# geopolars/geopolars

Hardware: AMD Instinct MI355X
Metric: predicate evals/sec (10M pts x 1k polys point-in-polygon) (higher is better)
Workload: dtype f64

## Files before the change

geopolars_amd/csrc/gpk_pipflow.hip:

```cpp
#include "gpk_pipshared.h"

namespace gpk {

constexpr int FLOW_P_MAX = 8;
constexpr int FLOW_BLOCK = 1024, FLOW_W = FLOW_BLOCK / 64;
constexpr int FLOW_ITEMS = 128;
constexpr int FLOW_PASS_AT = 40;
constexpr int FLOW_MAX_TILES = 1536;
constexpr int FLOW_ID_BITS = 22;
constexpr uint32_t FLOW_DEAD = 0xFFFFFFFFu;
constexpr uint32_t FLOW_MULTI = 0x80000000u;
constexpr uint32_t FLOW_PEND = FLOW_MULTI;
static_assert(64 * FLOW_P_MAX == 512, "an entry keeps the row within its tile in 9 bits");
static_assert(FLOW_MAX_TILES <= (1 << 14), "FlowItem::loc keeps the tile in 14 bits");

struct FlowItem {
    double px, py;
    uint32_t aux;
    uint32_t loc;
};
static_assert(sizeof(FlowItem) == 24, "list slot");

#ifdef GPK_TILE_TRACE
#define FLOW_STAMP(i)                                                                                                    \
    do {                                                                                                                 \
        if (h.stats && lane == 0 && wave % 5 == 0 && blockIdx.x < 900u) h.stats[8 + (blockIdx.x * 4 + wave / 5) * 16 + (i)] = wall_clock64(); \
    } while (0)
#if GPK_TILE_TRACE == 2
#define FLOW_PHASE(i)                                        \
    do {                                                     \
        asm volatile("s_waitcnt vmcnt(0) lgkmcnt(0)" ::: "memory"); \
        const unsigned long long _n = wall_clock64();        \
        g_phase[i] += _n - g_last;                           \
        g_last = _n;                                         \
    } while (0)
#define FLOW_PHASE_ARGS , unsigned long long (&g_phase)[6], unsigned long long& g_last
#define FLOW_PHASE_PASS , g_phase, g_last
#else
#define FLOW_PHASE(i) do {} while (0)
#define FLOW_PHASE_ARGS
#define FLOW_PHASE_PASS
#endif
#else
#define FLOW_STAMP(i) do {} while (0)
#define FLOW_PHASE(i) do {} while (0)
#define FLOW_PHASE_ARGS
#define FLOW_PHASE_PASS
#endif

#define H_COLD(field) (kernel_arg_at<decltype(ChainHot::field)>((uint32_t)offsetof(ChainHot, field)))
#define T_COLD(field) (kernel_arg_at<decltype(FusedTail::field)>((uint32_t)(sizeof(ChainHot) + offsetof(FusedTail, field))))
static_assert(sizeof(ChainHot) % 8 == 0, "FusedTail follows ChainHot in the argument segment");

__device__ __forceinline__ uint32_t cvt_u32_sat(double v) {
    uint32_t r;
    asm("v_cvt_u32_f64 %0, %1" : "=v"(r) : "v"(v));
    return r;
}
__device__ __forceinline__ void wave_lds_fence() {
    __builtin_amdgcn_fence(__ATOMIC_RELEASE, "wavefront");
    __builtin_amdgcn_wave_barrier();
    __builtin_amdgcn_fence(__ATOMIC_ACQUIRE, "wavefront");
}

__device__ __forceinline__ void ring_edge_flat(double sx, double sy, double ex, double ey, double cx, double cy, int& wn, bool& on, bool& unsure) {
    const bool up = sy <= cy && ey >= cy, down = sy > cy && ey <= cy;
    const bool left = cx < fmin(sx, ex), within = !left && cx <= fmax(sx, ex);
    const double detleft = (sx - cx) * (ey - cy), detright = (sy - cy) * (ex - cx);
    const double det = detleft - detright;
    const double errbound = 3.3306690738754716e-16 * (fabs(detleft) + fabs(detright));
    const bool opposite = (detleft > 0.0 && detright <= 0.0) || (detleft < 0.0 && detright >= 0.0) || detleft == 0.0;
    const bool certain = opposite || fabs(det) >= errbound;
    const bool eval = (up || down) && within;
    unsure |= eval && !certain;
    on |= eval && certain && det == 0.0;
    wn += (up && ey != cy && (left || (within && det > 0.0))) ? 1 : 0;
    wn -= (down && (left || (within && det < 0.0))) ? 1 : 0;
}

__device__ __forceinline__ void flow_settle(const ChainHot& h, uint32_t* s_ttot, uint32_t t, uint32_t slot, uint32_t row, uint32_t li, uint32_t cnt,
                                            uint32_t first) {
    if (cnt == 0u) {
        h.pool[slot] = FLOW_DEAD;
        if (h.counts) h.counts[row] = 0u;
        atomicSub(&s_ttot[t], 1u);
    } else if (cnt == 1u) {
        h.pool[slot] = (first << 9) | li;
    } else {
        h.pool[slot] = FLOW_MULTI | (cnt << 9) | li;
        if (h.counts) h.counts[row] = cnt;
        atomicAdd(&s_ttot[t], cnt - 1u);
    }
}

template <int TS>
__device__ __forceinline__ void flow_exact_pass(const ChainHot& h, FlowItem* items, uint32_t& n_list, int lane, uint32_t* s_ttot, uint32_t tile0) {
    const uint32_t n = n_list < 64u ? n_list : 64u;
    wave_lds_fence();
    const bool act = (uint32_t)lane < n;
    double qx = 0.0, qy = 0.0;
    uint32_t hd = 0u, loc = 0u;
    if (act) {
        const FlowItem* it = items + lane;
        qx = it->px;
        qy = it->py;
        hd = it->aux;
        loc = it->loc;
    }
    const int count = (int)(hd & HCHAIN_COUNT_MASK);
    const double2* __restrict__ v = H_COLD(chain_xy) + (hd >> HCHAIN_START_SHIFT);
    const int i1 = count < 1 ? count : 1, i2 = count < 2 ? count : 2, i3 = count < 3 ? count : 3, i4 = count < 4 ? count : 4;
    double2 a0 = v[0], a1 = v[i1], a2 = v[i2], a3 = v[i3], a4 = v[i4];
    asm volatile("" : "+v"(a0.x), "+v"(a0.y), "+v"(a1.x), "+v"(a1.y), "+v"(a2.x), "+v"(a2.y), "+v"(a3.x), "+v"(a3.y), "+v"(a4.x), "+v"(a4.y));
    int wn = ((int)(hd << (28 - HCHAIN_BASE_SHIFT))) >> 28;
    bool unsure = false, on = false;
    ring_edge_flat(a0.x, a0.y, a1.x, a1.y, qx, qy, wn, on, unsure);
    ring_edge_flat(a1.x, a1.y, a2.x, a2.y, qx, qy, wn, on, unsure);
    ring_edge_flat(a2.x, a2.y, a3.x, a3.y, qx, qy, wn, on, unsure);
    ring_edge_flat(a3.x, a3.y, a4.x, a4.y, qx, qy, wn, on, unsure);
    if (count > 4) {
        double ax = a4.x, ay = a4.y;
        for (int j = 4; j < count; ++j) {
            const double2 b = v[j + 1];
            on |= dev::ring_edge_filtered(ax, ay, b.x, b.y, qx, qy, wn, unsure);
            ax = b.x;
            ay = b.y;
        }
    }
    const bool walk = act && (count == 0 || unsure);
    const bool inside = !on && wn != 0;
    const uint32_t t = loc >> 18, li = loc & 511u;
    const uint32_t slot = ((tile0 + t) << TS) + ((loc >> 9) & 511u), row = ((tile0 + t) << TS) + li;
    if (act && !walk && !inside) flow_settle(h, s_ttot, t, slot, row, li, 0u, 0u);
    unsigned long long wm = __ballot(walk);
#ifdef GPK_TILE_TRACE
    unsigned long long* const stats = nullptr;
#else
    unsigned long long* const stats = H_COLD(stats);
#endif
    if (stats) {
        const unsigned long long edges = wave_sum_u64((unsigned long long)(act ? count : 0));
        if (lane == 0) {
            atomicAdd(&stats[0], (unsigned long long)n);
            atomicAdd(&stats[1], edges);
            if (wm) atomicAdd(&stats[2], (unsigned long long)__popcll(wm));
        }
    }
    while (wm) {
        const int j = __builtin_ctzll(wm);
        wm &= wm - 1ull;
        const double x = __shfl(qx, j, 64), y = __shfl(qy, j, 64);
        const unsigned long long cf = chain_generic_row_first_call(H_COLD(cold), x, y, lane);
        if (lane == j) flow_settle(h, s_ttot, t, slot, row, li, (uint32_t)cf, (uint32_t)(cf >> 32));
    }
    n_list -= n;
    if (n_list) {
        FlowItem keep{};
        if ((uint32_t)lane < n_list) keep = items[64 + lane];
        wave_lds_fence();
        if ((uint32_t)lane < n_list) items[lane] = keep;
    }
    wave_lds_fence();
}

typedef uint32_t u32x4 __attribute__((ext_vector_type(4)));

static __device__ __noinline__ void flow_settle_pending(const double2* pts_xy, const ChainCold* cold, uint32_t* pool, uint32_t* counts, unsigned long long* stats,
                                                        uint32_t* s_ttot, uint32_t t, uint32_t tile, uint32_t n_ent, int lane, int ts) {
    asm volatile("s_waitcnt vmcnt(0)" ::: "memory");
    uint32_t* seg = pool + ((size_t)tile << ts);
    for (uint32_t i = 0; i < n_ent; i += 64u) {
        const uint32_t e = i + (uint32_t)lane < n_ent ? __hip_atomic_load(seg + i + lane, __ATOMIC_RELAXED, __HIP_MEMORY_SCOPE_AGENT) : 0u;
        unsigned long long pm = __ballot((e & ~511u) == FLOW_PEND);
        while (pm) {
            const int j = __builtin_ctzll(pm);
            pm &= pm - 1ull;
            const uint32_t li = (uint32_t)__shfl((int)e, j, 64) & 511u, row = (tile << ts) + li, slot = i + (uint32_t)j;
            const double2 q = pts_xy[row];
            const unsigned long long cf = chain_generic_row_first_call(cold, q.x, q.y, lane);
            const uint32_t cnt = (uint32_t)cf, first = (uint32_t)(cf >> 32);
            if (lane == 0) {
                if (stats) atomicAdd(&stats[2], 1ull);
                if (cnt == 0u) {
                    seg[slot] = FLOW_DEAD;
                    if (counts) counts[row] = 0u;
                    atomicSub(&s_ttot[t], 1u);
                } else if (cnt == 1u) {
                    seg[slot] = (first << 9) | li;
                } else {
                    seg[slot] = FLOW_MULTI | (cnt << 9) | li;
                    if (counts) counts[row] = cnt;
                    atomicAdd(&s_ttot[t], cnt - 1u);
                }
            }
        }
    }
}

template <bool SIMPLE, bool FULL, int P>
__device__ __forceinline__ void flow_tile(const ChainHot& h, const uint2* s_mask, const uint32_t* s_rec0, FlowItem* items, uint32_t& n_list, uint32_t t,
                                          uint32_t tile0, int lane, uint32_t* s_tcand, uint32_t* s_ttot FLOW_PHASE_ARGS) {
    constexpr int S = PIP_SUB, FLOW_TILE = 64 * P, TS = P == 8 ? 9 : (P == 4 ? 8 : (P == 2 ? 7 : 6));
    static_assert(P == 1 || P == 2 || P == 4 || P == 8, "tile sizes");
    static_assert(S == 8, "the sub-cell arithmetic below is written for 8 x 8 sub-cells");
    asm volatile("" : "+v"(lane));
    const uint32_t tile = tile0 + t;
    const int64_t base = (int64_t)tile * FLOW_TILE;
    const int64_t n_points = FULL ? 0 : H_COLD(n_points);
    const uint32_t rem = FULL ? (uint32_t)FLOW_TILE : (uint32_t)(n_points - base < (int64_t)FLOW_TILE ? n_points - base : (int64_t)FLOW_TILE);
    double px[P], py[P];
    {
        const double2* __restrict__ tile_xy = h.pts_xy + base;
        static_for<P>([&](auto K) {
            constexpr int k = decltype(K)::value;
            double2 v = make_double2(NAN, NAN);
            if (FULL || ((uint32_t)(k * 64 + lane) < rem && dev::valid_row(H_COLD(pts_validity), base + k * 64 + lane))) v = dev::load_stream(tile_xy + (k * 64 + lane));
            px[k] = v.x;
            py[k] = v.y;
        });
    }
    GPK_SCHED_FENCE();
    FLOW_PHASE(1);
    const int logR = h.logR;
    const uint32_t sub_max = ((uint32_t)S << logR) - 1u;
    uint32_t sidx4[(P + 3) / 4], gw[P];
    u32x4 rec[P];
    static_for<(P + 3) / 4>([&](auto J) { sidx4[decltype(J)::value] = 0u; });
    uint32_t sxs[P], sys_[P], r0s[P];
    uint2 ms[P];
    static_for<P>([&](auto K) {
        constexpr int k = decltype(K)::value;
        uint32_t sx = cvt_u32_sat((px[k] - h.rx0) * h.inv_fw_s), sy = cvt_u32_sat((py[k] - h.ry0) * h.inv_fh_s);
        sx = sx < sub_max ? sx : sub_max;
        sy = sy < sub_max ? sy : sub_max;
        const uint32_t at = ((sy >> 3) << (logR - 5)) + (sx >> 8);
        ms[k] = s_mask[at];
        r0s[k] = s_rec0[at];
        sxs[k] = sx;
        sys_[k] = sy;
    });
    GPK_SCHED_FENCE();
    static_for<P>([&](auto K) {
        constexpr int k = decltype(K)::value;
        const uint32_t sx = sxs[k], sy = sys_[k], bit = (sx >> 3) & 31u;
        const bool real = !__builtin_isunordered(px[k], py[k]);
        const bool has = real && ((ms[k].x >> bit) & 1u) != 0u;
        const bool want = real && !has && ((ms[k].y >> bit) & 1u) != 0u;
        sidx4[k / 4] |= (((sy & 3u) << 3) | (sx & 7u)) << (8 * (k % 4));
        rec[k] = u32x4{0u, 0u, 0u, 0u};
        gw[k] = 0u;
        if (has) {
            const uint32_t w = r0s[k] + (uint32_t)__popc(__builtin_amdgcn_ubfe(ms[k].x, 0u, bit));
            rec[k] = *reinterpret_cast<const u32x4*>(h.half + (2u * w + ((sy >> 2) & 1u)));
        }
        if (want) gw[k] = h.cell[((sy >> 3) << logR) + (sx >> 3)];
    });
    GPK_SCHED_FENCE();
    FLOW_PHASE(2);
    uint32_t run = 0u, n_new = 0u;
    bool pend = false;
    uint32_t* const tile_counts = h.counts ? h.counts + base : nullptr;
    uint32_t* const tile_pool = h.pool + ((size_t)tile << TS);
    static_for<P>([&](auto K) {
        constexpr int k = decltype(K)::value;
        const uint32_t li = (uint32_t)(k * 64 + lane);
        const uint32_t s5 = (sidx4[k / 4] >> (8 * (k % 4))) & 31u;
        const uint32_t lw = (s5 & 16u) ? rec[k].y : rec[k].x;
        const uint32_t lab = (lw >> (2u * (s5 & 15u))) & 3u;
        uint32_t r = lab ? (rec[k].z & 0x3FFFFFFFu) : CODE_NONE;
        const uint32_t g = gw[k];
        const bool single = (g & 0xC0000001u) == 0x40000000u;
        if (single) r = (g >> 1) & 0x1FFFFFFFu;
        const bool walk = g != 0u && !single;
        if (!SIMPLE) {
            if (r != CODE_NONE) {
                const uint32_t geom = h.part_geom ? h.part_geom[r] : r;
                r = dev::valid_row(h.polys_validity, geom) ? geom : CODE_NONE;
            }
        }
        if (walk) r = 0u;
        const bool mine = FULL || li < rem;
        const bool cand = mine && r != CODE_NONE;
        bool listed = cand && (lab >= 2u || walk);
        const unsigned long long mcand = __ballot(cand);
        const uint32_t rank = run + lanes_below(mcand);
        uint32_t e = (r << 9) | li;
        unsigned long long ml = __ballot(listed);
        if (ml) {
            if (__builtin_expect(n_list + n_new + (uint32_t)__popcll(ml) > (uint32_t)FLOW_ITEMS, 0)) {
                if (listed && n_list + n_new + lanes_below(ml) >= (uint32_t)FLOW_ITEMS) {
                    listed = false;
                    e = FLOW_PEND | li;
                }
                ml = __ballot(listed);
                pend = true;
            }
            if (listed) {
                FlowItem* it = items + (n_list + n_new + lanes_below(ml));
                it->px = px[k];
                it->py = py[k];
                it->aux = walk ? 0u : rec[k].w;
                it->loc = (t << 18) | (rank << 9) | li;
            }
            n_new += (uint32_t)__popcll(ml);
        }
        if (tile_counts && mine) dev::store_stream(tile_counts + li, cand ? 1u : 0u);
        if (cand) tile_pool[rank] = e;
        run += (uint32_t)__popcll(mcand);
        GPK_SCHED_FENCE();
    });
    if (lane == 0) {
        s_tcand[t] = run;
        s_ttot[t] = run;
    }
    n_list += n_new;
    FLOW_PHASE(3);
    if (__builtin_expect(pend, 0)) flow_settle_pending(h.pts_xy, H_COLD(cold), h.pool, h.counts, H_COLD(stats), s_ttot, t, tile, run, lane, TS);
}

__device__ __forceinline__ void flow_emit_chunk(const ChainHot& h, uint32_t e, uint32_t row0, uint32_t pt0, unsigned long long* out64, uint32_t room, uint32_t& done,
                                                int lane) {
    const bool live = e != FLOW_DEAD;
    const bool multi = live && (e & FLOW_MULTI) != 0u;
    const unsigned long long mm = __ballot(multi);
    if (__builtin_expect(mm == 0ull, 1)) {
        const unsigned long long m = __ballot(live);
        const uint32_t at = done + lanes_below(m);
        if (live && at < room) __builtin_nontemporal_store(((unsigned long long)(e >> 9) << 32) | (unsigned long long)(row0 + (e & 511u)), out64 + at);
        done += (uint32_t)__popcll(m);
        return;
    }
    const uint32_t n_out = !live ? 0u : (multi ? (e >> 9) & ((1u << FLOW_ID_BITS) - 1u) : 1u);
    uint32_t incl = n_out;
#pragma unroll
    for (int o = 1; o < 64; o <<= 1) {
        const uint32_t v = __shfl_up(incl, o, 64);
        if (lane >= o) incl += v;
    }
    const uint32_t at = done + incl - n_out;
    if (live && !multi && at < room) __builtin_nontemporal_store(((unsigned long long)(e >> 9) << 32) | (unsigned long long)(row0 + (e & 511u)), out64 + at);
    unsigned long long wm = mm;
    while (wm) {
        const int j = __builtin_ctzll(wm);
        wm &= wm - 1ull;
        const uint32_t lj = (uint32_t)__shfl((int)e, j, 64) & 511u, aj = (uint32_t)__shfl((int)at, j, 64);
        const double2 q = h.pts_xy[pt0 + lj];
        chain_generic_row_call(H_COLD(cold), q.x, q.y, lane, reinterpret_cast<uint2*>(out64 + aj), aj < room ? room - aj : 0u, row0 + lj);
    }
    done += (uint32_t)__shfl((int)incl, 63, 64);
}

template <bool SIMPLE, int P>
__global__ __launch_bounds__(FLOW_BLOCK) void pip_tile_flow_kernel(ChainHot h, FusedTail tail) {
    constexpr int WORDS = PIP_ROUTE_RMAX * PIP_ROUTE_RMAX / 32, W = FLOW_W, TS = P == 8 ? 9 : (P == 4 ? 8 : (P == 2 ? 7 : 6));
    __shared__ uint2 s_mask[WORDS];
    __shared__ uint32_t s_rec0[WORDS];
    __shared__ FlowItem s_items[W][FLOW_ITEMS];
    __shared__ uint32_t s_tcand[FLOW_MAX_TILES], s_ttot[FLOW_MAX_TILES];
    __shared__ uint32_t s_next, s_next2, s_wg, s_wgtot, s_gave_up;
    __shared__ unsigned long long s_part[W];
    const int lane = threadIdx.x & 63, wave = __builtin_amdgcn_readfirstlane(threadIdx.x >> 6);
    FLOW_STAMP(0);
    unsigned long long my_ticket = 0ull;
    if (threadIdx.x == 0) my_ticket = __hip_atomic_fetch_add(T_COLD(ticket), 1ull, __ATOMIC_RELAXED, __HIP_MEMORY_SCOPE_AGENT);
    {
        const int R = H_COLD(R), words = R * R / 32;
        const uint4* __restrict__ src = reinterpret_cast<const uint4*>(H_COLD(route));
        for (int i = threadIdx.x; i < words; i += FLOW_BLOCK) {
            const uint4 rw = src[i];
            s_mask[i] = make_uint2(rw.x, rw.y);
            s_rec0[i] = rw.z;
        }
    }
    FLOW_STAMP(1);
    if (threadIdx.x == 0) {
        s_wg = (uint32_t)(my_ticket - T_COLD(ticket_base));
        s_next = 0u;
        s_next2 = 0u;
        s_gave_up = 0u;
    }
    __syncthreads();
    const uint32_t wg = __builtin_amdgcn_readfirstlane(s_wg);
    const uint32_t T0 = (uint32_t)((int64_t)wg * H_COLD(n_tiles) / (int64_t)gridDim.x), T1 = (uint32_t)((int64_t)(wg + 1u) * H_COLD(n_tiles) / (int64_t)gridDim.x);
    const uint32_t nt = T1 - T0;
    const bool want_pairs = T_COLD(pairs) != nullptr;
    FLOW_STAMP(2);
    const uint32_t nf = (int64_t)T1 <= (int64_t)H_COLD(n_full_tiles) ? nt : ((int64_t)T0 >= (int64_t)H_COLD(n_full_tiles) ? 0u : (uint32_t)(H_COLD(n_full_tiles) - (int32_t)T0));
    uint32_t n_list = 0u;
#ifdef GPK_TILE_TRACE
    int n_mine = 0;
#if GPK_TILE_TRACE == 2
    unsigned long long g_phase[6] = {0ull, 0ull, 0ull, 0ull, 0ull, 0ull}, g_last = wall_clock64();
#endif
#endif
    auto draw = [&](uint32_t* counter) -> uint32_t {
        __builtin_amdgcn_wave_barrier();
        const uint32_t d = __hip_atomic_fetch_add(counter, 1u, __ATOMIC_RELAXED, __HIP_MEMORY_SCOPE_WORKGROUP);
        return __builtin_amdgcn_readfirstlane(d) >> 6;
    };
    {
        uint32_t t = draw(&s_next);
        while (t < nf) {
            const uint32_t tn = draw(&s_next);
            FLOW_PHASE(4);
            if (n_list >= (uint32_t)FLOW_PASS_AT) flow_exact_pass<TS>(h, s_items[wave], n_list, lane, s_ttot, T0);
            FLOW_PHASE(0);
            flow_tile<SIMPLE, true, P>(h, s_mask, s_rec0, s_items[wave], n_list, t, T0, lane, s_tcand, s_ttot FLOW_PHASE_PASS);
            t = tn;
#if defined(GPK_TILE_TRACE) && GPK_TILE_TRACE != 2
            if (n_mine < 6) FLOW_STAMP(3 + n_mine);
            ++n_mine;
#endif
        }
    }
    for (;;) {
        const uint32_t t = draw(&s_next2) + nf;
        if (t >= nt) break;
        if (n_list >= (uint32_t)FLOW_PASS_AT) flow_exact_pass<TS>(h, s_items[wave], n_list, lane, s_ttot, T0);
        flow_tile<SIMPLE, false, P>(h, s_mask, s_rec0, s_items[wave], n_list, t, T0, lane, s_tcand, s_ttot FLOW_PHASE_PASS);
    }
    while (n_list) flow_exact_pass<TS>(h, s_items[wave], n_list, lane, s_ttot, T0);
#if defined(GPK_TILE_TRACE) && GPK_TILE_TRACE == 2
    FLOW_PHASE(5);
    if (h.stats && lane == 0 && wave % 5 == 0 && blockIdx.x < 900u)
        for (int i = 0; i < 6; ++i) h.stats[8 + (blockIdx.x * 4 + wave / 5) * 16 + 3 + i] = g_phase[i];
#endif
    FLOW_STAMP(9);
    __syncthreads();
    FLOW_STAMP(10);
    constexpr int EM_C = P < 4 ? P : 4, EM_T = 24 / EM_C;
    uint32_t ent[EM_T][EM_C], cand[EM_T];
    auto em_request = [&](uint32_t first) {
        static_for<EM_T>([&](auto Rr) {
            constexpr int r = decltype(Rr)::value;
            const uint32_t et = first + (uint32_t)(r * W);
            cand[r] = et < nt && want_pairs ? s_tcand[et] : 0u;
            cand[r] = __builtin_amdgcn_readfirstlane(cand[r]);
            const uint32_t* seg = h.pool + ((size_t)(T0 + et) << TS);
            static_for<EM_C>([&](auto Cc) {
                constexpr int c = decltype(Cc)::value;
                ent[r][c] = FLOW_DEAD;
                if ((uint32_t)(c * 64 + lane) < cand[r]) ent[r][c] = seg[c * 64 + lane];
            });
        });
    };
    em_request((uint32_t)wave);
    if (wave == 0) {
        uint32_t carry = 0u;
        for (uint32_t c0 = 0; c0 < nt; c0 += 64u) {
            const uint32_t v = c0 + (uint32_t)lane < nt ? s_ttot[c0 + lane] : 0u;
            uint32_t incl = v;
#pragma unroll
            for (int o = 1; o < 64; o <<= 1) {
                const uint32_t a = __shfl_up(incl, o, 64);
                if (lane >= o) incl += a;
            }
            if (c0 + (uint32_t)lane < nt) s_ttot[c0 + lane] = carry + incl - v;
            carry += (uint32_t)__shfl((int)incl, 63, 64);
        }
        if (lane == 0) s_wgtot = carry;
    }
    __syncthreads();
    const unsigned long long wg_tot = (unsigned long long)s_wgtot;
    const unsigned long long epoch = T_COLD(epoch);
    unsigned long long* const slots = T_COLD(slots);
    if (threadIdx.x == 0) __hip_atomic_store(&slots[wg], (epoch << FUSED_TOTAL_BITS) | wg_tot, __ATOMIC_RELAXED, __HIP_MEMORY_SCOPE_AGENT);
    unsigned long long acc = 0;
    bool gave_up = false;
    for (unsigned b = threadIdx.x; b < wg; b += FLOW_BLOCK) {
        unsigned long long v;
        uint32_t spins = 0;
        while (((v = __hip_atomic_load(&slots[b], __ATOMIC_RELAXED, __HIP_MEMORY_SCOPE_AGENT)) >> FUSED_TOTAL_BITS) != epoch) {
            __builtin_amdgcn_s_sleep(8);
            if (++spins > FUSED_SPIN_LIMIT) {
                gave_up = true;
                break;
            }
        }
        acc += v & ((1ull << FUSED_TOTAL_BITS) - 1ull);
    }
    if (gave_up) __hip_atomic_store(&s_gave_up, 1u, __ATOMIC_RELAXED, __HIP_MEMORY_SCOPE_WORKGROUP);
    acc = wave_sum_u64(acc);
    if (lane == 0) s_part[wave] = acc;
    __syncthreads();
    const bool lost = s_gave_up != 0u;
    unsigned long long base_off = 0;
#pragma unroll
    for (int w = 0; w < W; ++w) base_off += s_part[w];
    if ((wg == gridDim.x - 1 || lost) && threadIdx.x == 0) {
        unsigned long long* const lostp = T_COLD(lost);
        if (lost) __hip_atomic_store(lostp, epoch, __ATOMIC_RELAXED, __HIP_MEMORY_SCOPE_AGENT);
        const bool any_lost = lost || __hip_atomic_load(lostp, __ATOMIC_RELAXED, __HIP_MEMORY_SCOPE_AGENT) == epoch;
        unsigned long long* const grand = T_COLD(grand);
        unsigned long long* const grand_host = T_COLD(grand_host);
        *grand = any_lost ? FUSED_LOST : base_off + wg_tot;
        if (grand_host) *grand_host = any_lost ? FUSED_LOST : base_off + wg_tot;
    }
    FLOW_STAMP(11);
    if (!want_pairs || lost) return;
    unsigned long long* const pairs64 = reinterpret_cast<unsigned long long*>(T_COLD(pairs));
    const int64_t capacity = T_COLD(capacity);
    const uint32_t left_base = T_COLD(left_base);
    for (uint32_t first = (uint32_t)wave; first < nt; first += (uint32_t)(EM_T * W)) {
        if (first != (uint32_t)wave) em_request(first);
        static_for<EM_T>([&](auto Rr) {
            constexpr int r = decltype(Rr)::value;
            const uint32_t et = first + (uint32_t)(r * W);
            if (cand[r]) {
                const unsigned long long off = base_off + (unsigned long long)s_ttot[et];
                unsigned long long* const out64 = pairs64 + off;
                const int64_t left = capacity - (int64_t)off;
                const uint32_t room = left <= 0 ? 0u : (left > (int64_t)0xFFFFFFFFll ? 0xFFFFFFFFu : (uint32_t)left);
                const uint32_t pt0 = (T0 + et) << TS, row0 = pt0 + left_base;
                uint32_t done = 0u;
                static_for<EM_C>([&](auto Cc) {
                    constexpr int c = decltype(Cc)::value;
                    if ((uint32_t)(c * 64) < cand[r]) flow_emit_chunk(h, ent[r][c], row0, pt0, out64, room, done, lane);
                });
                if (EM_C * 64 < 64 * P) {
                    const uint32_t* seg = h.pool + ((size_t)(T0 + et) << TS);
                    for (uint32_t i = (uint32_t)(EM_C * 64); i < cand[r]; i += 64u) {
                        const uint32_t e = i + (uint32_t)lane < cand[r] ? seg[i + lane] : FLOW_DEAD;
                        flow_emit_chunk(h, e, row0, pt0, out64, room, done, lane);
                    }
                }
            }
        });
    }
    FLOW_STAMP(12);
}

int pip_flow_points_per_lane(int64_t n_left_rows, int64_t n_right_geoms, int32_t R, int wgs) {
    if (R < 32 || R > PIP_ROUTE_RMAX || wgs < 1) return 0;
    if (n_right_geoms >= (int64_t)((1u << FLOW_ID_BITS) - 1u)) return 0;
    if (n_left_rows >= (int64_t)0xFFFFFE00ll) return 0;
    static const int forced = [] {
        const char* e = getenv("GPK_FLOW_P");
        return e ? atoi(e) : 0;
    }();
    const int64_t waves = (int64_t)wgs * FLOW_W;
    for (int p = FLOW_P_MAX; p >= 1; p >>= 1) {
        const int64_t n_tiles = (n_left_rows + 64 * p - 1) / (64 * p);
        if ((n_tiles + wgs - 1) / wgs > (int64_t)FLOW_MAX_TILES) return p == FLOW_P_MAX ? 0 : 2 * p;
        if (forced ? p == forced : (n_tiles >= waves || p == 1)) return p;
    }
    return 1;
}
size_t pip_flow_pool_bytes(int64_t n_left_rows) { return sizeof(uint32_t) * (size_t)((n_left_rows + 511) / 512) * 512u; }

template <int P>
static int32_t launch_pip_flow_p(const ChainHot& hot, const FusedTail& tail, int wgs, hipStream_t s) {
    if (hot.part_geom == nullptr && hot.polys_validity == nullptr)
        GPK_LAUNCH("gpk_pip_tile", (pip_tile_flow_kernel<true, P>), dim3((unsigned)wgs), dim3(FLOW_BLOCK), 0, s, hot, tail);
    else
        GPK_LAUNCH("gpk_pip_tile", (pip_tile_flow_kernel<false, P>), dim3((unsigned)wgs), dim3(FLOW_BLOCK), 0, s, hot, tail);
    return GPK_OK;
}
int32_t launch_pip_flow(const ChainHot& hot, const FusedTail& tail, int wgs, int points_per_lane, hipStream_t s) {
    switch (points_per_lane) {
        case 8: return launch_pip_flow_p<8>(hot, tail, wgs, s);
        case 4: return launch_pip_flow_p<4>(hot, tail, wgs, s);
        case 2: return launch_pip_flow_p<2>(hot, tail, wgs, s);
        case 1: return launch_pip_flow_p<1>(hot, tail, wgs, s);
    }
    return fail(GPK_ERR_INVALID_ARGUMENT, "spatial_join: %d points per lane", points_per_lane);
}

}
```

Before: 115100 billion.

## Split exact pass into issue/finish to overlap edge loads with tile point loads

Splits the per-tile flow into a point-load request and a decide step. The deferred exact pass is split into an issue phase and a finish phase: the issue phase compacts the list and issues loads of up to four chain edges for short-chain items, then the next tile's point loads are issued, and the finish phase evaluates those edges. Items whose chains are longer, and results that are unsure, are pushed back onto the list for the full exact pass. This is meant to hide global-memory latency of the edge fetches behind the streaming point loads, at the cost of extra register pressure and added list-compaction work.

```diff
diff --git a/geopolars_amd/csrc/gpk_pipflow.hip b/geopolars_amd/csrc/gpk_pipflow.hip
--- a/geopolars_amd/csrc/gpk_pipflow.hip
+++ b/geopolars_amd/csrc/gpk_pipflow.hip
@@ -155,12 +155,139 @@
     }
     n_list -= n;
     if (n_list) {
-        FlowItem keep{};
-        if ((uint32_t)lane < n_list) keep = items[64 + lane];
+        const bool more = (uint32_t)lane < n_list;
+        double kx = 0.0, ky = 0.0;
+        uint32_t kaux = 0u, kloc = 0u;
+        if (more) {
+            const FlowItem* it = items + 64 + lane;
+            kx = it->px;
+            ky = it->py;
+            kaux = it->aux;
+            kloc = it->loc;
+        }
         wave_lds_fence();
-        if ((uint32_t)lane < n_list) items[lane] = keep;
+        if (more) {
+            FlowItem* it = items + lane;
+            it->px = kx;
+            it->py = ky;
+            it->aux = kaux;
+            it->loc = kloc;
+        }
     }
     wave_lds_fence();
+}
+
+struct FlowPass {
+    double2 a0, a1, a2, a3, a4;
+    double qx, qy;
+    uint32_t hd, loc;
+};
+constexpr uint32_t FLOW_SLOW_AT = 16;
+
+template <int TS>
+__device__ __forceinline__ void flow_pass_issue(const ChainHot& h, FlowItem* items, uint32_t& n_list, int lane, uint32_t* s_ttot, uint32_t tile0, FlowPass& ps) {
+    const uint32_t n = n_list < 64u ? n_list : 64u;
+    wave_lds_fence();
+    const bool act = (uint32_t)lane < n;
+    double qx = 0.0, qy = 0.0;
+    uint32_t aux = 0u, loc = 0u;
+    if (act) {
+        const FlowItem* it = items + lane;
+        qx = it->px;
+        qy = it->py;
+        aux = it->aux;
+        loc = it->loc;
+    }
+    const bool fast = act && (aux & HCHAIN_COUNT_MASK) - 1u < 4u;
+    const bool slow = act && !fast;
+    const unsigned long long ms = __ballot(slow);
+    const uint32_t rest = n_list - n, ns = (uint32_t)__popcll(ms);
+    if (rest | ns) {
+        const bool more = (uint32_t)lane < rest;
+        double kx = 0.0, ky = 0.0;
+        uint32_t kaux = 0u, kloc = 0u;
+        if (more) {
+            const FlowItem* it = items + 64 + lane;
+            kx = it->px;
+            ky = it->py;
+            kaux = it->aux;
+            kloc = it->loc;
+        }
+        wave_lds_fence();
+        if (slow) {
+            FlowItem* it = items + lanes_below(ms);
+            it->px = qx;
+            it->py = qy;
+            it->aux = aux;
+            it->loc = loc;
+        }
+        if (more) {
+            FlowItem* it = items + ns + lane;
+            it->px = kx;
+            it->py = ky;
+            it->aux = kaux;
+            it->loc = kloc;
+        }
+        wave_lds_fence();
+    }
+    n_list = ns + rest;
+    ps.qx = qx;
+    ps.qy = qy;
+    ps.hd = fast ? aux : 0u;
+    ps.loc = loc;
+    if (__builtin_expect(ns >= FLOW_SLOW_AT, 0)) flow_exact_pass<TS>(h, items, n_list, lane, s_ttot, tile0);
+    const int count = (int)(ps.hd & HCHAIN_COUNT_MASK);
+    const double2* __restrict__ v = H_COLD(chain_xy) + (ps.hd >> HCHAIN_START_SHIFT);
+    const int i1 = count < 1 ? count : 1, i2 = count < 2 ? count : 2, i3 = count < 3 ? count : 3;
+    ps.a0 = v[0];
+    ps.a1 = v[i1];
+    ps.a2 = v[i2];
+    ps.a3 = v[i3];
+    ps.a4 = v[count];
+}
+
+template <int TS>
+__device__ __forceinline__ void flow_pass_finish(const ChainHot& h, FlowItem* items, uint32_t& n_list, int lane, uint32_t* s_ttot, uint32_t tile0, FlowPass& ps) {
+    double2 a0 = ps.a0, a1 = ps.a1, a2 = ps.a2, a3 = ps.a3, a4 = ps.a4;
+    asm volatile("" : "+v"(a0.x), "+v"(a0.y), "+v"(a1.x), "+v"(a1.y), "+v"(a2.x), "+v"(a2.y), "+v"(a3.x), "+v"(a3.y), "+v"(a4.x), "+v"(a4.y));
+    const uint32_t hd = ps.hd, loc = ps.loc;
+    const double qx = ps.qx, qy = ps.qy;
+    const bool act = hd != 0u;
+    int wn = ((int)(hd << (28 - HCHAIN_BASE_SHIFT))) >> 28;
+    bool unsure = false, on = false;
+    ring_edge_flat(a0.x, a0.y, a1.x, a1.y, qx, qy, wn, on, unsure);
+    ring_edge_flat(a1.x, a1.y, a2.x, a2.y, qx, qy, wn, on, unsure);
+    ring_edge_flat(a2.x, a2.y, a3.x, a3.y, qx, qy, wn, on, unsure);
+    ring_edge_flat(a3.x, a3.y, a4.x, a4.y, qx, qy, wn, on, unsure);
+    const bool redo = act && unsure;
+    const bool inside = !on && wn != 0;
+    const uint32_t t = loc >> 18, li = loc & 511u;
+    const uint32_t slot = ((tile0 + t) << TS) + ((loc >> 9) & 511u), row = ((tile0 + t) << TS) + li;
+    if (act && !redo && !inside) flow_settle(h, s_ttot, t, slot, row, li, 0u, 0u);
+#ifdef GPK_TILE_TRACE
+    unsigned long long* const stats = nullptr;
+#else
+    unsigned long long* const stats = H_COLD(stats);
+#endif
+    if (stats) {
+        const unsigned long long settled = __ballot(act && !redo);
+        const unsigned long long edges = wave_sum_u64((unsigned long long)(hd & HCHAIN_COUNT_MASK));
+        if (lane == 0) {
+            atomicAdd(&stats[0], (unsigned long long)__popcll(settled));
+            atomicAdd(&stats[1], edges);
+        }
+    }
+    const unsigned long long mr = __ballot(redo);
+    if (__builtin_expect(mr != 0ull, 0)) {
+        if (redo) {
+            FlowItem* it = items + (n_list + lanes_below(mr));
+            it->px = qx;
+            it->py = qy;
+            it->aux = 0u;
+            it->loc = loc;
+        }
+        n_list += (uint32_t)__popcll(mr);
+    }
 }
 
 typedef uint32_t u32x4 __attribute__((ext_vector_type(4)));
@@ -197,28 +324,35 @@
     }
 }
 
+template <bool FULL, int P>
+__device__ __forceinline__ void flow_tile_request(const ChainHot& h, uint32_t t, uint32_t tile0, int lane, double (&px)[P], double (&py)[P]) {
+    constexpr int FLOW_TILE = 64 * P;
+    static_assert(P == 1 || P == 2 || P == 4 || P == 8, "tile sizes");
+    asm volatile("" : "+v"(lane));
+    const int64_t base = (int64_t)(tile0 + t) * FLOW_TILE;
+    const int64_t n_points = FULL ? 0 : H_COLD(n_points);
+    const uint32_t rem = FULL ? (uint32_t)FLOW_TILE : (uint32_t)(n_points - base < (int64_t)FLOW_TILE ? n_points - base : (int64_t)FLOW_TILE);
+    const double2* __restrict__ tile_xy = h.pts_xy + base;
+    static_for<P>([&](auto K) {
+        constexpr int k = decltype(K)::value;
+        double2 v = make_double2(NAN, NAN);
+        if (FULL || ((uint32_t)(k * 64 + lane) < rem && dev::valid_row(H_COLD(pts_validity), base + k * 64 + lane))) v = dev::load_stream(tile_xy + (k * 64 + lane));
+        px[k] = v.x;
+        py[k] = v.y;
+    });
+    GPK_SCHED_FENCE();
+}
+
 template <bool SIMPLE, bool FULL, int P>
-__device__ __forceinline__ void flow_tile(const ChainHot& h, const uint2* s_mask, const uint32_t* s_rec0, FlowItem* items, uint32_t& n_list, uint32_t t,
-                                          uint32_t tile0, int lane, uint32_t* s_tcand, uint32_t* s_ttot FLOW_PHASE_ARGS) {
+__device__ __forceinline__ void flow_tile_decide(const ChainHot& h, const uint2* s_mask, const uint32_t* s_rec0, FlowItem* items, uint32_t& n_list, uint32_t t,
+                                                 uint32_t tile0, int lane, uint32_t* s_tcand, uint32_t* s_ttot, double (&px)[P], double (&py)[P] FLOW_PHASE_ARGS) {
     constexpr int S = PIP_SUB, FLOW_TILE = 64 * P, TS = P == 8 ? 9 : (P == 4 ? 8 : (P == 2 ? 7 : 6));
-    static_assert(P == 1 || P == 2 || P == 4 || P == 8, "tile sizes");
     static_assert(S == 8, "the sub-cell arithmetic below is written for 8 x 8 sub-cells");
     asm volatile("" : "+v"(lane));
     const uint32_t tile = tile0 + t;
     const int64_t base = (int64_t)tile * FLOW_TILE;
     const int64_t n_points = FULL ? 0 : H_COLD(n_points);
     const uint32_t rem = FULL ? (uint32_t)FLOW_TILE : (uint32_t)(n_points - base < (int64_t)FLOW_TILE ? n_points - base : (int64_t)FLOW_TILE);
-    double px[P], py[P];
-    {
-        const double2* __restrict__ tile_xy = h.pts_xy + base;
-        static_for<P>([&](auto K) {
-            constexpr int k = decltype(K)::value;
-            double2 v = make_double2(NAN, NAN);
-            if (FULL || ((uint32_t)(k * 64 + lane) < rem && dev::valid_row(H_COLD(pts_validity), base + k * 64 + lane))) v = dev::load_stream(tile_xy + (k * 64 + lane));
-            px[k] = v.x;
-            py[k] = v.y;
-        });
-    }
     GPK_SCHED_FENCE();
     FLOW_PHASE(1);
     const int logR = h.logR;
@@ -403,9 +537,17 @@
         while (t < nf) {
             const uint32_t tn = draw(&s_next);
             FLOW_PHASE(4);
-            if (n_list >= (uint32_t)FLOW_PASS_AT) flow_exact_pass<TS>(h, s_items[wave], n_list, lane, s_ttot, T0);
+            double px[P], py[P];
+            if (n_list >= (uint32_t)FLOW_PASS_AT) {
+                FlowPass ps;
+                flow_pass_issue<TS>(h, s_items[wave], n_list, lane, s_ttot, T0, ps);
+                flow_tile_request<true, P>(h, t, T0, lane, px, py);
+                flow_pass_finish<TS>(h, s_items[wave], n_list, lane, s_ttot, T0, ps);
+            } else {
+                flow_tile_request<true, P>(h, t, T0, lane, px, py);
+            }
             FLOW_PHASE(0);
-            flow_tile<SIMPLE, true, P>(h, s_mask, s_rec0, s_items[wave], n_list, t, T0, lane, s_tcand, s_ttot FLOW_PHASE_PASS);
+            flow_tile_decide<SIMPLE, true, P>(h, s_mask, s_rec0, s_items[wave], n_list, t, T0, lane, s_tcand, s_ttot, px, py FLOW_PHASE_PASS);
             t = tn;
 #if defined(GPK_TILE_TRACE) && GPK_TILE_TRACE != 2
             if (n_mine < 6) FLOW_STAMP(3 + n_mine);
@@ -416,8 +558,16 @@
     for (;;) {
         const uint32_t t = draw(&s_next2) + nf;
         if (t >= nt) break;
-        if (n_list >= (uint32_t)FLOW_PASS_AT) flow_exact_pass<TS>(h, s_items[wave], n_list, lane, s_ttot, T0);
-        flow_tile<SIMPLE, false, P>(h, s_mask, s_rec0, s_items[wave], n_list, t, T0, lane, s_tcand, s_ttot FLOW_PHASE_PASS);
+        double px[P], py[P];
+        if (n_list >= (uint32_t)FLOW_PASS_AT) {
+            FlowPass ps;
+            flow_pass_issue<TS>(h, s_items[wave], n_list, lane, s_ttot, T0, ps);
+            flow_tile_request<false, P>(h, t, T0, lane, px, py);
+            flow_pass_finish<TS>(h, s_items[wave], n_list, lane, s_ttot, T0, ps);
+        } else {
+            flow_tile_request<false, P>(h, t, T0, lane, px, py);
+        }
+        flow_tile_decide<SIMPLE, false, P>(h, s_mask, s_rec0, s_items[wave], n_list, t, T0, lane, s_tcand, s_ttot, px, py FLOW_PHASE_PASS);
     }
     while (n_list) flow_exact_pass<TS>(h, s_items[wave], n_list, lane, s_ttot, T0);
 #if defined(GPK_TILE_TRACE) && GPK_TILE_TRACE == 2
```

Result: no change. 115700 billion, median of 6 (+0.5%).
